# LeadRDRK/ZPack

Measured on AMD Instinct MI355X. Metric: decompressed GiB/s over all entries; % HBM roofline, higher is better.
Workload: dtype u8; 1 GPU; c2_lz4_64k; entries_per_gpu=100000, entries_total=100000, archive_image_bytes_this_rank=3543588472, archive_image_bytes_all_ranks=3543588472, method=lz4, level=0, class_mix=70/20/5/5 text/records/random/runs, parallelism=one batch per rank, no data-path collective, rehearsal_one_card=False, frames_by=liblz4/libzstd of the image, reference writer call sequence

## Files before the change

zpack_amd/csrc/lz4_wave.h:

```cpp
#pragma once
#include "zpk_device.h"
#include "xxh3_device.h"
#include "seq_exec.h"

namespace zpk {

__device__ __noinline__ u32 window_word(const u8* a, const u8* lo, const u8* hi)
{
    if (a >= lo && a + 4 <= hi) return ld32(a);
    u32 v = 0;
    #pragma unroll
    for (int i = 0; i < 4; i++) if (a + i >= lo && a + i < hi) v |= (u32)ld8(a + i) << (8 * i);
    return v;
}

struct ByteWindow {
    u32 w;
    const u8* base;
    const u8* lo;
    const u8* hi;

    __device__ __forceinline__ void load(const u8* p, int lane)
    {
        base = (const u8*)((u64)p & ~(u64)3);
        w = window_word(base + 4 * lane, lo, hi);
    }
    __device__ __forceinline__ u32 byte(const u8* p, int lane)
    {
        u64 d = (u64)(p - base);
        if (d >= 256) { load(p, lane); d = (u64)(p - base); }
        u32 word = (u32)__builtin_amdgcn_readlane((int)w, (int)(d >> 2));
        return (word >> (8 * (d & 3))) & 0xFF;
    }
};

struct DecodeOut { int rc; u64 produced; };

struct Lz4Resume { u64 ip_off, op_off, frame_ip_off, frame_op_off; u32 in_blocks, nframes; };

#ifndef LZ4W_SEG
#define LZ4W_SEG 60u
#endif
static_assert(LZ4W_SEG <= 64u, "the visited-position mask of a segment is one 64-bit word");
#define LZ4W_CHUNK (64u * LZ4W_SEG)
#define LZ4W_SLACK 64u
#ifndef LZ4W_RUNIN
#define LZ4W_RUNIN LZ4W_SEG
#endif

#ifndef LZ4W_FIX_CONT
#define LZ4W_FIX_CONT 1
#endif

#ifndef LZ4W_SPLIT_FIRST
#define LZ4W_SPLIT_FIRST 0
#endif
#ifndef LZ4W_NREC
#define LZ4W_NREC 576u
#endif
struct alignas(16) Lz4WaveShared {
    u8  stage[LZ4W_CHUNK + LZ4W_SLACK + 16];
    u16 rec[LZ4W_NREC];
};

struct Lz4Bytes {
    lds_cp8 S;
    const u8* g;
    u32 cbase, cend;
    __device__ __forceinline__ u32 at(u32 pos) const
    {
        if (pos < cend) return lds_ld8(S + (pos - cbase));
        return (u32)ld8(g + pos);
    }
    __device__ __forceinline__ u32 at16(u32 pos) const
    {
        if (pos + 1 < cend) return lds_ld16(S + (pos - cbase));
        return at(pos) | (at(pos + 1) << 8);
    }
};

struct Lz4Tok { u32 next, lit_pos, lit, ml, off, flags; };

__device__ __forceinline__ Lz4Tok lz4_token_at(const Lz4Bytes& B, u32 p, u32 C, bool want_offset)
{
    Lz4Tok t; t.flags = 0; t.ml = 0; t.off = 1;
    const u32 tok = B.at(p);
    u32 q = p + 1, lit = tok >> 4;
    if (lit == 15) {
        u32 b;
        do {
            if (q >= C) { t.flags = 1; t.next = C; t.lit = 0; t.lit_pos = q; return t; }
            b = B.at(q++); lit += b;
        } while (b == 255 && lit < 0x7F000000u);
        if (b == 255) { t.flags = 1; t.next = C; t.lit = 0; t.lit_pos = q; return t; }
    }
    t.lit_pos = q; t.lit = lit;
    if (lit > C - q) { t.flags = 1; t.next = C; return t; }
    q += lit;
    if (q == C) { t.flags = 2; t.next = C; return t; }
    if (C - q < 2) { t.flags = 5; t.next = C; return t; }
    if (want_offset) t.off = B.at16(q);
    q += 2;
    u32 ml = tok & 15;
    if (ml == 15) {
        u32 b;
        do {
            if (q >= C) { t.flags = 5; t.next = C; return t; }
            b = B.at(q++); ml += b;
        } while (b == 255 && ml < 0x7F000000u);
        if (b == 255) { t.flags = 5; t.next = C; return t; }
    }
    t.ml = ml + 4;
    t.next = q;
    return t;
}

struct Lz4Quick { u32 lit_pos, lit, ml, next, off, slow; };
__device__ __forceinline__ u32 lt31(u32 a, u32 b) { return (a - b) >> 31; }
__device__ __forceinline__ Lz4Quick lz4_quick(lds_cp8 S, u32 cbase, u32 p, u32 lim)
{
    const lds_cp8 at = S + (p - cbase);
    const u32 tok = lds_ld8(at), b1 = lds_ld8(at + 1);
    const u32 lit4 = tok >> 4, mlc = tok & 15;
    const u32 le = (lit4 + 1) >> 4, me = (mlc + 1) >> 4;
    const u32 lit = lit4 + (b1 & (0u - le));
    const u32 q = 1 + le + lit;
    const u32 b2 = lds_ld8(at + q + 2);
    Lz4Quick r;
    r.off = lds_ld16(at + q);
    r.lit_pos = p + 1 + le; r.lit = lit;
    r.ml = mlc + 4 + (b2 & (0u - me));
    r.next = p + q + 2 + me;
    r.slow = (le & ((b1 + 1) >> 8)) | (me & ((b2 + 1) >> 8)) | lt31(lim, p + q + 3);
    return r;
}

struct Lz4Walk { u32 exit, flags; u64 m; };
template <bool FIRST>
__device__ __forceinline__ Lz4Walk lz4_walk(const Lz4Bytes& B, bool on, u32 from, u32 seg_start, u32 seg_end, u32 C,
                                            const Lz4Walk& old, u32& entry_out, SeqStats& stt)
{
    (void)stt;
    const u32 lim = B.cend < C ? B.cend : C;
    const i32 seg_len = (i32)(seg_end - seg_start), lim_rel = (i32)(lim - seg_start);
    const lds_cp8 base = B.S + (seg_start - B.cbase);
    const bool start_in = on && (i32)(from - seg_start) < seg_len;
    i32 rp = start_in ? (i32)(from - seg_start) : seg_len;
    bool live = start_in;
    u32 flags = 0, exit_far = from, far = on && !start_in ? 1u : 0u;
    u64 m = 0;
    for (;;) {
        live = live && rp < seg_len;
        const bool inseg = FIRST ? rp >= 0 : true;
        if (!FIRST) {
            live = live && !((u32)(old.m >> (rp & 63)) & 1u);
        }
        if (__builtin_amdgcn_ballot_w64(live) == 0) break;
        SEQ_STAT(if (FIRST) stt.hops_first++; else stt.hops_fix++);
        m |= (u64)((live && inseg) ? 1u : 0u) << (rp & 63);
        const lds_cp8 at = base + rp;
        const u32 tok = lds_ld8(at), b1 = lds_ld8(at + 1);
        const u32 lit4 = tok >> 4, mlc = tok & 15;
        const bool l15 = lit4 == 15, m15 = mlc == 15;
        const u32 q = lit4 + 1 + (l15 ? b1 + 1 : 0u);
        const u32 b2 = lds_ld8(at + q + 2);
        const i32 n2 = rp + (i32)q + 2;
        i32 nx = n2 + (m15 ? 1 : 0);
        const bool slow = (l15 && b1 == 255) || (m15 && b2 == 255) || n2 >= lim_rel;
        if (live && slow) {
            SEQ_STAT(stt.slow_hops++);
            const Lz4Tok tt = lz4_token_at(B, seg_start + (u32)rp, C, false);
            nx = (i32)(tt.next - seg_start);
            if (tt.flags && !inseg) nx = 0;
            else if (tt.flags || nx >= seg_len) { flags |= tt.flags; far = 1; exit_far = tt.next; nx = seg_len; }
        }
        rp = live ? nx : rp;
    }
    Lz4Walk w; w.m = m; w.flags = flags; w.exit = far ? exit_far : seg_start + (u32)rp;
    if (!FIRST && rp < seg_len) {
        const u64 tail = old.m & ~((1ull << (rp & 63)) - 1);
        w.m |= tail;
        w.flags |= old.flags;
        w.exit = old.exit;
    }
    if (!on) w = old;
    entry_out = !FIRST ? from : m ? seg_start + (u32)__ffsll((long long)m) - 1u : w.exit;
    return w;
}

struct Lz4NoEmit { __device__ __forceinline__ int operator()(const SeqBatch&, int, u32) const { return D_OK; } };

template <int COOP = 2, bool EMIT = false, class Emit = Lz4NoEmit>
__device__ inline int lz4_block_wave(Lz4WaveShared& sh, Watchdog& wd, SeqStats& stt, const u8* ip, u32 C, const u8* rd_hi,
                                     u8* dst_lo, u8*& op_io, u8* oend, int lane, Emit emit = Emit())
{
    u8* op = op_io;
    if (C == 0) return D_MALFORMED;
    u32 cpos = 0;
    bool finished = false;
    while (!finished) {
        if (wd.expired()) return D_MALFORMED;
        const u64 tp0 = SEQ_T(); (void)tp0;
        if (cpos >= C) return D_MALFORMED;
        const u32 nst = C - cpos < LZ4W_CHUNK + LZ4W_SLACK ? C - cpos : LZ4W_CHUNK + LZ4W_SLACK;
        const u32 tok_end = C - cpos < LZ4W_CHUNK ? C : cpos + LZ4W_CHUNK;
        wave_mem_fence();
        if (ip + cpos + ((nst + 15u) & ~15u) <= rd_hi) {
            const u8* const g = ip + cpos + 16u * (u32)lane;
            ZPK_LDS u8* const d0 = (ZPK_LDS u8*)sh.stage;
            #pragma unroll
            for (u32 i = 0; i < LZ4W_CHUNK + LZ4W_SLACK; i += WAVE * 16)
                if (i + 16u * (u32)lane < nst) __builtin_amdgcn_global_load_lds((const ZPK_GLOBAL u32*)(g + i), (ZPK_LDS u32*)(d0 + i), 16, 0, 0);
            asm volatile("s_waitcnt vmcnt(0)" ::: "memory");
        } else {
            for (u32 i = (u32)lane * 16; i < nst; i += WAVE * 16) {
                const u8* g = ip + cpos + i;
                if (i + 16 <= nst && g + 16 <= rd_hi) { u128 v = ld128(g); __builtin_memcpy(sh.stage + i, &v, 16); }
                else for (u32 k = i; k < nst && k < i + 16; k++) sh.stage[k] = ld8(ip + cpos + k);
            }
        }
        __builtin_amdgcn_fence(__ATOMIC_ACQ_REL, "workgroup");
        u64 ts = SEQ_T(); (void)ts; SEQ_STAT(stt.t_stage += ts - tp0; stt.chunks++);
        Lz4Bytes B; B.S = to_lds(sh.stage); B.g = ip; B.cbase = cpos; B.cend = cpos + nst;
        const u32 lim = B.cend < C ? B.cend : C;
        const u32 my_start = cpos + (u32)lane * LZ4W_SEG;
        const u32 my_end = my_start + LZ4W_SEG < tok_end ? my_start + LZ4W_SEG : tok_end;
        const bool active = my_start < tok_end;
        u32 my_entry = my_start;
        Lz4Walk w; w.exit = my_start; w.flags = 0; w.m = 0;
        w = lz4_walk<true>(B, active, lane == 0 ? my_start : (my_start - cpos > LZ4W_RUNIN ? my_start - LZ4W_RUNIN : cpos), my_start, my_end, C, w, my_entry, stt);
        SEQ_STAT({ u64 t2 = SEQ_T(); stt.t_walk1 += t2 - ts; ts = t2; });
#if LZ4W_FIX_CONT
        {
            static_assert(sizeof(sh.rec) >= 16 * (WAVE + 1), "65 records of 16 bytes (lane 63 reads a slot nobody uses)");
            const lds_p8 slot = to_lds_rw((u8*)sh.rec) + 16u * (u32)lane;
            const auto pack = [](const Lz4Walk& a) { u128 v; v.lo = a.m; v.hi = ((u64)a.flags << 32) | a.exit; return v; };
            const auto unpack = [](const u128& v) { Lz4Walk a; a.m = v.lo; a.exit = (u32)v.hi; a.flags = (u32)(v.hi >> 32); return a; };
            if (lane == 0) my_entry = w.exit;
            bool on = false;
            for (int iter = 0; iter < 2 * 66;) {
                const bool step2 = iter & 1;
                const u32 s0 = my_start + (step2 ? LZ4W_SEG : 0u);
                const u32 s1 = s0 + LZ4W_SEG < C ? s0 + LZ4W_SEG : C;
                const u32 next_end = s1 + LZ4W_SEG < C ? s1 + LZ4W_SEG : C;
                u32 from; Lz4Walk old;
                wave_mem_fence();
                if (!step2) {
                    SEQ_STAT(stt.fix_iters++);
                    from = (u32)__shfl_up((int)w.exit, 1, 64);
                    on = active && from != my_entry;
                    if (__ballot(on) == 0) break;
                    old = w;
                    lds_st128(slot, pack(w));
                } else {
                    from = w.exit;
                    old = unpack(lds_ld128(slot + 16));
                    wave_mem_fence();
                    lds_st128(slot, pack(w));
                }
                wave_mem_fence();
                u32 unused;
                const Lz4Walk r = lz4_walk<false>(B, on, from, s0, s1, C, old, unused, stt);
                if (!step2) {
                    my_entry = on ? from : my_entry;
                    on = on && r.exit != w.exit && r.exit < next_end && r.exit - cpos < LZ4W_CHUNK;
                    w = r;
                    iter += __ballot(on) != 0 ? 1 : 2;
                } else {
                    const u32 hn = (u32)__shfl_up((int)from, 1, 64);
                    const bool got = ((__ballot(on) << 1) >> lane) & 1;
                    wave_mem_fence();
                    if (on) lds_st128(slot + 16, pack(r));
                    wave_mem_fence();
                    w = unpack(lds_ld128(slot));
                    my_entry = got ? hn : my_entry;
                    iter++;
                }
            }
        }
#else
        for (int iter = 0; iter < 66; iter++) {
            SEQ_STAT(stt.fix_iters++);
            u32 e = (u32)__shfl_up((int)w.exit, 1, 64);
            if (lane == 0) e = cpos;
            const bool changed = active && e != my_entry;
            if (__ballot(changed) == 0) break;
            u32 unused;
            w = lz4_walk<false>(B, changed, e, my_start, my_end, C, w, unused, stt);
            my_entry = changed ? e : my_entry;
        }
#endif
        SEQ_STAT({ u64 t2 = SEQ_T(); stt.t_fix += t2 - ts; ts = t2; });
        if (!active) { w.exit = (u32)__shfl((int)w.exit, 63, 64); }
        const u64 lastmask = __ballot(active);
        const int last_lane = 63 - __clzll((long long)lastmask);
        const u32 chain_exit = (u32)__builtin_amdgcn_readlane((int)w.exit, last_lane);
        const u32 fl = (u32)__ballot(active && (w.flags & 1)) != 0 || (__ballot(active && (w.flags & 1)) >> 32) != 0 ? 1u : 0u;
        if (__ballot(active && (w.flags & 2)) != 0) finished = true;
        const u32 my_nseq = active ? (u32)__popcll(w.m) : 0u;
        const u32 x = wave_scan_add(my_nseq);
        const u32 nseq = (u32)__builtin_amdgcn_readlane((int)x, 63);
        SEQ_STAT({ u64 t2 = SEQ_T(); stt.t_emit += t2 - ts; stt.t_parse += t2 - tp0; });
        const u8* ipb = ip;
        asm volatile("" : "+s"(ipb));
        Lz4Bytes Bb = B; Bb.g = ipb;
        ZPK_LDS u16* const rec = (ZPK_LDS u16*)sh.rec;
        for (u32 b0 = 0, bstep; b0 < nseq; b0 += bstep) {
            bstep = LZ4W_SPLIT_FIRST && b0 < WAVE ? WAVE / 2 : WAVE;
            const u32 bw = b0 % LZ4W_NREC;
            if (bw == 0) {
                wave_mem_fence();
                u64 m = w.m;
                u32 k = x - my_nseq;
                const u32 rel = my_start - cpos;
                while (m) {
                    const u32 b = (u32)__ffsll((long long)m) - 1u;
                    m &= m - 1;
                    if (k - b0 < LZ4W_NREC) rec[k - b0] = (u16)(rel + b);
                    k++;
                }
                if (active && x == nseq && nseq - b0 < LZ4W_NREC)
                    rec[nseq - b0] = (u16)(w.exit - cpos < LZ4W_CHUNK + LZ4W_SLACK ? w.exit - cpos : LZ4W_CHUNK + LZ4W_SLACK);
                wave_mem_fence();
            }
            const int cnt = (int)(nseq - b0 < bstep ? nseq - b0 : bstep);
            const u64 tq0 = SEQ_T(); (void)tq0;
            SeqBatch q; q.lit = ipb; q.lit_lds = SEQ_NO_LDS; q.ll = 0; q.ml = 0; q.off = 1; q.bad = 0;
            u32 tok_pos = cpos;
            if (lane < cnt) {
                const u32 p = cpos + (u32)rec[bw + (u32)lane];
                tok_pos = p;
                const Lz4Quick t = lz4_quick(B.S, B.cbase, p, lim);
                if (!t.slow) {
                    q.lit = ipb + t.lit_pos; q.ll = t.lit; q.ml = t.ml; q.off = t.off;
                } else {
                    const Lz4Tok tt = lz4_token_at(Bb, p, C, true);
                    q.lit = ipb + tt.lit_pos; q.ll = tt.lit; q.ml = tt.ml; q.off = tt.off;
                    if (tt.flags & 1) q.bad = (tt.flags & 4) ? 2u : 1u;
                }
                if (q.ll > (1u << 23)) q.ll = 1u << 23;
                if (q.ml > (1u << 23)) q.ml = 1u << 23;
                const u32 lp = (u32)(q.lit - ipb);
                if (q.ll <= SEQ_OWN_MAX && lp + q.ll <= B.cend) q.lit_lds = lp - B.cbase;
            }
            SEQ_STAT({ u64 t2 = SEQ_T(); stt.t_parse += t2 - tq0; stt.t_tok += t2 - tq0; });
            u32 dead = 0;
            if constexpr (!EMIT) {
                const u32 nx = bw + (u32)cnt;
                const u32 own = tok_pos - cpos;
#ifdef LZ4W_ROOM_OWN_TOKEN
                (void)nx; const u32 nxt = 0u;
#else
                const u32 nxt = (u32)rec[nx == LZ4W_NREC ? 0u : nx];
#endif
                dead = (u32)__builtin_amdgcn_readfirstlane((int)(nxt > own ? nxt : own));
            }
            int rc;
            if constexpr (EMIT) { (void)dead; rc = emit(q, cnt, (u32)(q.lit - ipb)); }
            else rc = seq_exec_batch<true, COOP, SEQ_ASM_LONG_LIT != 0>(q, cnt, op, oend, dst_lo, -1, lane, stt, B.S, to_lds_rw(sh.stage), dead);
            if (rc != D_OK) { op_io = op; return rc; }
        }
        if (fl) return D_MALFORMED;
        if (!finished && chain_exit <= cpos) return D_MALFORMED;
        cpos = chain_exit;
    }
    if (cpos != C) return D_MALFORMED;
    op_io = op;
    return D_OK;
}

template <int COOP = 2>
__device__ inline DecodeOut lz4f_decode_wave(Lz4WaveShared& sh, Watchdog& wd, SeqStats& stt, const u8* src, u64 src_size, const u8* src_lo, const u8* src_hi,
                                             u8* dst, u64 dst_cap, int lane, Lz4Resume* rs = nullptr)
{
    DecodeOut r; r.rc = D_OK; r.produced = 0;
    const u8* ip = src;
    const u8* const iend = src + src_size;
    u8* op = dst;
    u8* const oend = dst + dst_cap;
    bool resume_in_blocks = false, first = true;
    if (rs && (rs->in_blocks || rs->nframes)) {
        ip = src + rs->frame_ip_off; op = dst + rs->frame_op_off;
        resume_in_blocks = rs->in_blocks != 0;
        first = rs->nframes == 0;
    }
    for (;; first = false) {
        if (wd.expired()) { r.rc = D_MALFORMED; return r; }
        if (!first && (ip == iend || op == oend)) break;
        if (rs) { rs->frame_ip_off = (u64)(ip - src); rs->frame_op_off = (u64)(op - dst); if (!resume_in_blocks) rs->in_blocks = 0; }
        if (iend - ip < 7) { r.rc = D_TRUNCATED; r.produced = (u64)(op - dst); return r; }
        const u32 magic = uld32(ip);
        if ((magic & 0xFFFFFFF0u) == 0x184D2A50u) {
            if (iend - ip < 8) { r.rc = D_TRUNCATED; r.produced = (u64)(op - dst); return r; }
            const u64 sz = uld32(ip + 4);
            if ((u64)(iend - ip) - 8 < sz) { r.rc = D_TRUNCATED; r.produced = (u64)(op - dst); return r; }
            ip += 8 + sz;
            if (rs) rs->nframes++;
            continue;
        }
        if (magic != 0x184D2204u) { r.rc = D_MALFORMED; return r; }
        const u32 flg = uld8(ip + 4), bd = uld8(ip + 5);
        const bool indep = (flg >> 5) & 1, bck = (flg >> 4) & 1, has_cs = (flg >> 3) & 1, cck = (flg >> 2) & 1, has_dict = flg & 1;
        if ((flg >> 6) != 1 || (flg & 2)) { r.rc = D_MALFORMED; return r; }
        const u32 hdr = 7 + (has_cs ? 8 : 0) + (has_dict ? 4 : 0);
        if ((u64)(iend - ip) < hdr) { r.rc = D_TRUNCATED; r.produced = (u64)(op - dst); return r; }
        if (bd & 0x8F) { r.rc = D_MALFORMED; return r; }
        const u32 bcode = (bd >> 4) & 7;
        if (bcode < 4) { r.rc = D_MALFORMED; return r; }
        const u64 bmax = (u64)1 << (8 + 2 * bcode);
        u64 content_size = 0;
        if (has_cs) content_size = uni64(ld64(ip + 6));
        {
            u32 h = 0;
            lane0_guard();
            if (lane == 0) h = (xxh32_serial(ip + 4, hdr - 5, 0) >> 8) & 0xFF;
            if (uni(h) != uld8(ip + hdr - 1)) { r.rc = D_MALFORMED; return r; }
        }
        ip += hdr;

        u8* const frame_out = op;
        if (resume_in_blocks) { ip = src + rs->ip_off; op = dst + rs->op_off; resume_in_blocks = false; }
        for (;;) {
            if (wd.expired()) { r.rc = D_MALFORMED; return r; }
            if (rs) { rs->in_blocks = 1; rs->ip_off = (u64)(ip - src); rs->op_off = (u64)(op - dst); }
            if (iend - ip < 4) { r.rc = D_TRUNCATED; r.produced = (u64)(op - dst); return r; }
            const u32 bh = uld32(ip);
            ip += 4;
            if (bh == 0) break;
            const bool raw = bh >> 31;
            const u64 bsz = bh & 0x7FFFFFFFu;
            if (bsz > bmax) { r.rc = D_MALFORMED; return r; }
            if ((u64)(iend - ip) < bsz + (bck ? 4u : 0u)) {
                if (raw && !rs) {
                    u64 n = (u64)(iend - ip); if (n > bsz) n = bsz;
                    bool full = n > (u64)(oend - op);
                    if (full) n = (u64)(oend - op);
                    for (u64 i = (u64)lane * 16; i < n; i += WAVE * 16) gcopy_upto16(op + i, ip + i, (u32)(n - i < 16 ? n - i : 16));
                    op += n;
                    if (full) { r.rc = D_DST_FULL; r.produced = (u64)(op - dst); return r; }
                }
                r.rc = D_TRUNCATED; r.produced = (u64)(op - dst); return r;
            }
// ... 93 lines not shown
```

zpack_amd/csrc/seq_exec.h:

```cpp
#pragma once
#include "zpk_device.h"

namespace zpk {

__device__ __forceinline__ void gcopy_upto16(u8* d, const u8* s, u32 n)
{
    if (n >= 16) { st128(d, ld128(s)); return; }
    if (n & 8) { st64(d, ld64(s)); d += 8; s += 8; }
    if (n & 4) { st32(d, ld32(s)); d += 4; s += 4; }
    if (n & 2) { st16(d, ld16(s)); d += 2; s += 2; }
    if (n & 1) st8(d, ld8(s));
}

struct Copy32 { u128 lo, hi; };

__device__ __forceinline__ Copy32 gload_upto32(const u8* s, u32 n)
{
    Copy32 c; c.lo.lo = c.lo.hi = c.hi.lo = c.hi.hi = 0;
    if (n >= 16)      { c.lo = ld128(s); c.hi = ld128(s + n - 16); }
    else if (n >= 8)  { c.lo.lo = ld64(s); c.hi.lo = ld64(s + n - 8); }
    else if (n >= 4)  { c.lo.lo = ld32(s); c.hi.lo = ld32(s + n - 4); }
    else if (n >= 2)  { c.lo.lo = ld16(s); c.hi.lo = ld16(s + n - 2); }
    else if (n == 1)  { c.lo.lo = ld8(s); }
    return c;
// ... 80 lines not shown
    if (n > 48) gstore_upto16(d + 48, v3, n - 48);
}

__device__ __forceinline__ void gcopy_upto32(u8* d, const u8* s, u32 n)
{
    const Copy32 c = gload_upto32(s, n);
    gstore_upto32(d, c, n);
}

__device__ __forceinline__ const u8* readlane_ptr(const u8* p, int k)
{
    return (const u8*)(((u64)(u32)__builtin_amdgcn_readlane((int)(u32)((u64)p >> 32), k) << 32) |
                       (u32)__builtin_amdgcn_readlane((int)(u32)(u64)p, k));
}

__device__ __forceinline__ u8* shfl_ptr(const u8* p, int k)
{
    return (u8*)(((u64)(u32)__shfl((int)(u32)((u64)p >> 32), k, 64) << 32) | (u32)__shfl((int)(u32)(u64)p, k, 64));
}

__device__ __forceinline__ void coop_copy_rows(u64 mask, u32 n, u8* d, const u8* s, bool pat, u32 period, u64 pv, int lane)
{
    const int g = lane >> 4;
    const u32 sub16 = 16u * (u32)(lane & 15);
    while (mask) {
        int k[4];
        #pragma unroll
        for (int i = 0; i < 4; i++) { k[i] = mask ? __ffsll((long long)mask) - 1 : -1; if (mask) mask &= mask - 1; }
        const int kk = g == 0 ? k[0] : (g == 1 ? k[1] : (g == 2 ? k[2] : k[3]));
        const int from = kk < 0 ? lane : kk;
        const u32 rn_any = (u32)__shfl((int)n, from, 64);
        const u32 rn = kk < 0 ? 0u : rn_any;
        u8* const rd = shfl_ptr(d, from);
        const u8* const rs = shfl_ptr(s, from);
        const bool rpat = __shfl((int)(pat ? 1 : 0), from, 64) != 0;
        const u32 rper = (u32)__shfl((int)period, from, 64);
        u64 x = ((u64)(u32)__shfl((int)(u32)(pv >> 32), from, 64) << 32) | (u32)__shfl((int)(u32)pv, from, 64);
        if (rper < 8u) { x &= 0xFFFFFFFFull; x |= x << 32; }
        if (rper < 4u) { x &= 0x0000FFFF0000FFFFull; x |= x << 16; }
        if (rper < 2u) { x &= 0x00FF00FF00FF00FFull; x |= x << 8; }
        for (u32 c = sub16; __ballot(c < rn) != 0; c += 256u) {
            if (c < rn) {
                u128 v; v.lo = x; v.hi = x;
                if (!rpat) v = gload_upto16(rs + c, rn - c);
                gstore_upto16(rd + c, v, rn - c);
            }
        }
    }
}

__device__ __forceinline__ void seq_coop_round(u64 cm, u32 ml, u32 off, u8* ms, const u8* srcp, const u8* oend, int lane)
{
    const bool mine = (cm >> lane) & 1;
    const bool self_overlap = ml > off;
    const bool pat = mine && self_overlap && off <= 8u && (off & (off - 1u)) == 0u;
    Copy32 cb; cb.lo.lo = cb.lo.hi = cb.hi.lo = cb.hi.hi = 0;
    if (pat) cb = gload_wide32(srcp, off, srcp + 16 <= oend);
    const u64 gm = __ballot(mine && (pat || !self_overlap));
    if (gm) coop_copy_rows(gm, ml, ms, srcp, pat, off, cb.lo.lo, lane);
    u64 rest = cm & ~gm;
    while (rest) {
        const int k = __ffsll((long long)rest) - 1;
        rest &= rest - 1;
        const u32 n = (u32)__builtin_amdgcn_readlane((int)ml, k);
        const u32 koff = (u32)__builtin_amdgcn_readlane((int)off, k);
        u8* p = (u8*)readlane_ptr(ms, k);
        const u8* m = readlane_ptr(srcp, k);
        if (koff >= 16) {
            for (u32 c = (u32)lane * 16; c < koff; c += WAVE * 16) gcopy_upto16(p + c, m + c, koff - c);
            wave_mem_fence();
            for (u32 base = koff; base < n; base += koff) {
                const u32 slab = n - base < koff ? n - base : koff;
                for (u32 c = (u32)lane * 16; c < slab; c += WAVE * 16) gcopy_upto16(p + base + c, p + base - koff + c, slab - c);
                wave_mem_fence();
            }
        } else {
            for (u32 c = lane; c < n; c += WAVE) st8(p + c, ld8(m + c % koff));
        }
    }
}

#ifdef ZPK_STATS
struct SeqStats { u64 t_parse, t_lit, t_dep, t_rounds; u32 rounds, batches, coops, redirects; u64 t_stage, t_walk1, t_fix, t_emit, t_tok; u32 fix_iters, chunks, asm_batches, hops_first, hops_fix, slow_hops;
    u32 r_room, r_piece, r_both, r_straddle, k_lit, k_match, k_so16, k_so1; u64 t_asm, t_dir; u32 b_asm, b_dir; };
#define SEQ_T() __builtin_amdgcn_s_memtime()
#define SEQ_STAT(x) do { x; } while (0)
#else
struct SeqStats { };
#define SEQ_T() 0ull
#define SEQ_STAT(x) do { } while (0)
#endif

#define SEQ_OWN_MAX 32u
#ifndef SEQ_DEP_ROUNDS
#define SEQ_DEP_ROUNDS 4
#endif

#define SEQ_NO_LDS 0xFFFFFFFFu
#ifndef SEQ_ASM_LONG_LIT
#define SEQ_ASM_LONG_LIT 1
#endif
#define SEQ_ASM_PRE 32u
#define SEQ_ASM_SLACK 16u
struct SeqBatch {
    const u8* lit;
    u32 lit_lds;
    u32 ll, ml;
    u32 off;
    u32 bad;
};

template <typename S>
__device__ __forceinline__ u64 seq_dependencies(bool has_match, u32 r_ms, u32 r_me, u32 off, u32 need_len, u64 pending, int lane,
                                                i64& src_out, SeqStats& stt)
{
    (void)stt;
    S src = (S)r_ms - (S)off;
    u64 need = 0;
    const S send0 = src + (S)need_len;
    const bool reads_batch = has_match && send0 > 0;
    if (pending && __ballot(reads_batch) != 0) {
        int inside = -1;
        int klo = 0, khi = 0;
        #pragma unroll
        for (int step = 32; step >= 1; step >>= 1) {
            const u32 a = (u32)__shfl((int)r_me, klo + step - 1, 64);
            const u32 b = (u32)__shfl((int)r_ms, khi + step - 1, 64);
            if ((S)a <= src) klo += step;
            if ((S)b < send0) khi += step;
        }
        if (reads_batch && klo < khi) {
            if (khi > lane) khi = lane;
            const u64 span = (khi >= 64 ? ~0ull : ((1ull << khi) - 1)) & ~((1ull << klo) - 1);
            need = span & pending;
            if (need && (need & (need - 1)) == 0) inside = __ffsll((long long)need) - 1;
        }
        {
            const int probe = inside < 0 ? lane : inside;
            const u32 kms = (u32)__shfl((int)r_ms, probe, 64);
            const u32 knl = (u32)__shfl((int)need_len, probe, 64);
            if (inside >= 0 && !((S)kms <= src && send0 <= (S)kms + (S)knl)) inside = -1;
        }
        #pragma unroll 1
        for (int round = 0; round < SEQ_DEP_ROUNDS; round++) {
            if (__ballot(inside >= 0) == 0) break;
            SEQ_STAT(stt.redirects += (u32)__popcll(__ballot(inside >= 0)));
            const int probe = inside < 0 ? lane : inside;
            const S my_delta = (S)r_ms - src;
            const u32 dlo = (u32)__shfl((int)(u32)(u64)(i64)my_delta, probe, 64);
            const u32 dhi = sizeof(S) == 8 ? (u32)__shfl((int)(u32)((u64)(i64)my_delta >> 32), probe, 64) : 0u;
            const u32 nlo = (u32)__shfl((int)(u32)need, probe, 64), nhi = (u32)__shfl((int)(u32)(need >> 32), probe, 64);
            const int kin = __shfl(inside, probe, 64);
            if (inside >= 0) { src -= sizeof(S) == 8 ? (S)(i64)(((u64)dhi << 32) | dlo) : (S)(i32)dlo; need = ((u64)nhi << 32) | nlo; inside = kin; }
        }
    }
    src_out = (i64)src;
    return need;
}

template <bool NARROW_ONLY = false, int COOP = 2, bool LONG_LIT = false>
__device__ __forceinline__ int seq_exec_batch(const SeqBatch& q, int cnt, u8*& op, u8* oend, const u8* dst_lo, int lit_rle, int lane,
                                              SeqStats& stt, lds_cp8 lit_stage = nullptr, lds_p8 asm_buf = nullptr, u32 asm_cap = 0)
{
    u64 t0 = SEQ_T(); (void)t0; (void)stt;
    const u64 tb = t0; (void)tb;
    SEQ_STAT(stt.batches++);
    const bool act = lane < cnt;
    const u32 ll = act ? q.ll : 0u, ml = act ? q.ml : 0u;
    const u32 x = wave_scan_add(ll + ml);
    const u64 total = (u32)__builtin_amdgcn_readlane((int)x, 63);
    u8* const o = op + (x - (ll + ml));
    u8* const ms = o + ll;
    const bool has_match = act && ml != 0;
    {
        const u64 cap = (u64)(oend - op);
        const bool off_bad = has_match && (q.off == 0 || (u64)q.off > (u64)(ms - dst_lo));
        u32 v = 0;
        if (act) {
            if (q.bad == 1) v = 1;
            else if ((u64)(x - ml) > cap) v = 2;
            else if (q.bad == 2 || off_bad) v = 1;
            else if ((u64)x > cap) v = 2;
        }
        const u64 vm = __ballot(v != 0);
        if (vm != 0) return (u32)__builtin_amdgcn_readlane((int)v, __ffsll((long long)vm) - 1) == 1u ? D_MALFORMED : D_DST_FULL;
    }
    u64 pending = __ballot(has_match);

    const u32 r_ms = (u32)(ms - op), r_me = r_ms + ml;
    const u32 need_len = ml < q.off ? ml : q.off;
    i64 src;
    u64 need;
    if (NARROW_ONLY) need = seq_dependencies<i32>(has_match, r_ms, r_me, q.off, need_len, pending, lane, src, stt);
    else {
        const bool narrow = total < (1u << 30) && __ballot(has_match && q.off >= (1u << 30)) == 0;
        need = narrow ? seq_dependencies<i32>(has_match, r_ms, r_me, q.off, need_len, pending, lane, src, stt)
                      : seq_dependencies<i64>(has_match, r_ms, r_me, q.off, need_len, pending, lane, src, stt);
    }
    const u8* const srcp = op + src;
    const bool self_overlap = ml > need_len;
    const bool coop = has_match && (ml > SEQ_OWN_MAX || self_overlap);
    const bool early = has_match && !coop && src + (i64)need_len <= 0;
    SEQ_STAT({ u64 t1 = SEQ_T(); stt.t_dep += t1 - t0; t0 = t1; });

#ifdef ZPK_STATS
        if (lit_rle < 0 && NARROW_ONLY) {
            const bool fits = total + (SEQ_ASM_PRE + SEQ_ASM_SLACK) <= (u64)asm_cap;
            const u64 kl = __ballot(ll > SEQ_OWN_MAX), km = __ballot(has_match && !self_overlap && ml > SEQ_OWN_MAX);
            const u64 k16 = __ballot(has_match && self_overlap && q.off >= 16u), k1 = __ballot(has_match && self_overlap && q.off < 16u);
            const bool piece = ((LONG_LIT ? 0ull : kl) | km | k16 | k1) != 0;
            if (!fits) { if (piece) stt.r_both++; else stt.r_room++; }
            else {
                if (piece) stt.r_piece++;
                else if (__ballot(has_match && !early && src < 0) != 0 && (u64)(op - dst_lo) < SEQ_ASM_PRE) stt.r_straddle++;
                stt.k_lit += kl != 0; stt.k_match += km != 0; stt.k_so16 += k16 != 0; stt.k_so1 += k1 != 0;
            }
        }
#endif
    if (lit_rle < 0 && total + (SEQ_ASM_PRE + SEQ_ASM_SLACK) <= (u64)asm_cap) {
        const bool straddle = has_match && !early && src < 0;
        const u64 sm = __ballot(straddle);
        if (__ballot(coop || (!LONG_LIT && ll > SEQ_OWN_MAX)) == 0 && (sm == 0 || (u64)(op - dst_lo) >= SEQ_ASM_PRE)) {
            SEQ_STAT(stt.asm_batches++);
            const lds_p8 ob = asm_buf + SEQ_ASM_PRE;
            if (sm != 0 && lane < 2) lds_st128(asm_buf + 16 * lane, ld128(op - SEQ_ASM_PRE + 16 * lane));
            const u32 ln = LONG_LIT && ll > SEQ_OWN_MAX ? 0u : ll;
            Copy32 ca;
            if (q.lit_lds != SEQ_NO_LDS) {
                ca.lo.lo = ca.lo.hi = ca.hi.lo = ca.hi.hi = 0;
                if (ln) { ca.lo = lds_ld128(lit_stage + q.lit_lds); if (ln > 16) ca.hi = lds_ld128(lit_stage + q.lit_lds + (ln - 16)); }
            } else ca = gload_wide32(q.lit, ln, false);
            if (LONG_LIT && ll > SEQ_OWN_MAX) {
                const lds_p8 p = ob + (r_ms - ll);
                for (u32 c = 0; c < ll; c += 16) {
                    const u32 at = c + 16 <= ll ? c : ll - 16;
                    lds_st128(p + at, ld128(q.lit + at));
                }
            }
            const u32 mn = early ? ml : 0u;
            const Copy32 cb = gload_wide32(srcp, mn, srcp + 16 <= oend);
            lds_store_wide32(ob + (r_ms - ll), ca, ln);
            lds_store_wide32(ob + r_ms, cb, mn);
            wave_mem_fence();
            u64 done = ~pending | __ballot(early);
            pending &= ~done;
            u32 guard = 0;
            while (pending) {
                const bool ready = has_match && ((pending >> lane) & 1) && (need & ~done) == 0;
                const u64 rmask = __ballot(ready);
                if (rmask == 0 || ++guard > 70) return D_MALFORMED;
                SEQ_STAT(stt.rounds++);
                if (ready) {
                    const lds_cp8 sp = (lds_cp8)(ob + (i32)src);
                    Copy32 c; c.hi.lo = c.hi.hi = 0;
                    c.lo = lds_ld128(sp);
                    if (ml > 16) c.hi = lds_ld128(sp + (ml - 16));
                    lds_store_wide32(ob + r_ms, c, ml);
                }
                wave_mem_fence();
                done |= rmask;
                pending &= ~rmask;
            }
            const u32 tot = (u32)total;
            for (u32 c = (u32)lane * 16; c < tot; c += WAVE * 16) {
                const u128 v = lds_ld128((lds_cp8)(ob + c));
                if (c + 16 <= tot) st128(op + c, v);
                else gstore_upto16(op + c, v, tot - c);
            }
            wave_mem_fence();
            SEQ_STAT({ stt.t_asm += SEQ_T() - tb; stt.b_asm += (u32)total; });
            op += total;
            return D_OK;
        }
    }

    if (lit_rle >= 0) {
        if (__ballot(ll > SEQ_OWN_MAX) == 0) { for (u32 c = 0; c < ll; c++) st8(o + c, (u8)lit_rle); }
        else {
            for (int k = 0; k < cnt; k++) {
                const u32 n = (u32)__builtin_amdgcn_readlane((int)ll, k);
                u8* p = (u8*)readlane_ptr(o, k);
                for (u32 c = lane; c < n; c += WAVE) st8(p + c, (u8)lit_rle);
            }
        }
        if (early) { const Copy32 cb = gload_wide32(srcp, ml, srcp + 16 <= oend); gstore_wide32(ms, cb, ml); }
    } else {
        const bool long_lit = ll > SEQ_OWN_MAX;
        const u32 ln = long_lit ? 0u : ll, mn = early ? ml : 0u;
        Copy32 ca;
        const bool from_lds = q.lit_lds != SEQ_NO_LDS;
        if (from_lds) {
            ca.lo.lo = ca.lo.hi = ca.hi.lo = ca.hi.hi = 0;
            if (ln) { ca.lo = lds_ld128(lit_stage + q.lit_lds); if (ln > 16) ca.hi = lds_ld128(lit_stage + q.lit_lds + (ln - 16)); }
        } else ca = gload_wide32(q.lit, ln, false);
        const Copy32 cb = gload_wide32(srcp, mn, srcp + 16 <= oend);
        gstore_wide32(o, ca, ln);
        gstore_wide32(ms, cb, mn);
        if constexpr (COOP >= 2) {
            const u64 lm = __ballot(long_lit);
            if (lm) coop_copy_rows(lm, ll, o, q.lit, false, 16u, 0ull, lane);
        } else {
        u64 lm = __ballot(long_lit);
        while (lm) {
            const int k = __ffsll((long long)lm) - 1;
            lm &= lm - 1;
            const u32 n = (u32)__builtin_amdgcn_readlane((int)ll, k);
            u8* p = (u8*)readlane_ptr(o, k);
            const u8* s = readlane_ptr(q.lit, k);
            for (u32 c = (u32)lane * 16; c < n; c += WAVE * 16) gcopy_upto16(p + c, s + c, n - c);
        }
        }
    }
    wave_mem_fence();
    u64 done = ~pending | __ballot(early);
    pending &= ~done;
    SEQ_STAT({ u64 t1 = SEQ_T(); stt.t_lit += t1 - t0; t0 = t1; });

    u32 guard = 0;
    while (pending) {
        const bool ready = has_match && ((pending >> lane) & 1) && (need & ~done) == 0;
        const u64 rmask = __ballot(ready);
        if (rmask == 0 || ++guard > 70) return D_MALFORMED;
        SEQ_STAT(stt.rounds++);
        if (ready && !coop) {
            const Copy32 cb = gload_wide32(srcp, ml, srcp + 16 <= oend);
            gstore_wide32(ms, cb, ml);
        }
        if constexpr (COOP >= 1) {
            const u64 cm = __ballot(ready && coop);
            SEQ_STAT(stt.coops += (u32)__popcll(cm));
            if (cm) seq_coop_round(cm, ml, q.off, ms, srcp, oend, lane);
        } else {
        u64 cm = __ballot(ready && coop);
        SEQ_STAT(stt.coops += (u32)__popcll(cm));
        while (cm) {
            const int k = __ffsll((long long)cm) - 1;
            cm &= cm - 1;
            const u32 n = (u32)__builtin_amdgcn_readlane((int)ml, k);
            const u32 koff = (u32)__builtin_amdgcn_readlane((int)q.off, k);
            u8* p = (u8*)readlane_ptr(ms, k);
            const u8* m = readlane_ptr(srcp, k);
            if (koff >= n) { for (u32 c = (u32)lane * 16; c < n; c += WAVE * 16) gcopy_upto16(p + c, m + c, n - c); }
            else if (koff >= 16) {
                for (u32 c = (u32)lane * 16; c < koff; c += WAVE * 16) gcopy_upto16(p + c, m + c, koff - c);
                wave_mem_fence();
                for (u32 base = koff; base < n; base += koff) {
                    const u32 slab = n - base < koff ? n - base : koff;
                    for (u32 c = (u32)lane * 16; c < slab; c += WAVE * 16) gcopy_upto16(p + base + c, p + base - koff + c, slab - c);
                    wave_mem_fence();
                }
            } else {
                for (u32 c = lane; c < n; c += WAVE) st8(p + c, ld8(m + c % koff));
            }
// ... 13 lines not shown
```

zpack_amd/csrc/zpk_codec.hip:

```cpp
#include <hip/hip_runtime.h>
#include <stdio.h>
#include <stdlib.h>
#include <string.h>
#include <new>
#include <time.h>
#include <pthread.h>
#include <thread>
#include <atomic>
#include <vector>
#include <algorithm>


#include "zpk_device.h"
#include "xxh3_device.h"
#include "xxh3_span.h"
#include "lz4_wave.h"
#include "lx_ring.h"
#ifndef LX_WAVES_PER_SIMD
#define LX_WAVES_PER_SIMD 6
#endif
#include "zstd_wg.h"
#include "zstd_fse4.h"
#include "zstd_ring.h"
#include "lz4_pj.h"
// ... 159 lines not shown

template <bool LDS_KEYS = false>
__device__ __forceinline__ void finish_entry(const zpk_decode_desc& d, zpk_decode_result* res, u32 e, int status, u32 detail,
                                             u64 produced, const u8* out, int lane, lds_p8 sec = nullptr)
{
    u64 h = 0;
    lane0_guard();
    if (status == R_OK) {
        wave_mem_fence();
        h = xxh3_64_wave<LDS_KEYS>(out, d.uncomp_size, lane, sec);
        if (h != d.expect_hash && !(d.flags & ZPK_DF_SKIP_HASH)) status = R_FILE_HASH_MISMATCH;
    }
    lane0_guard();
    if (lane == 0) {
        zpk_decode_result r; r.status = status; r.detail = detail; r.produced = produced; r.hash = h;
        res[e] = r;
    }
}

__global__ __launch_bounds__(256) void k_stored(const u8* __restrict__ src, const zpk_decode_desc* __restrict__ desc,
                                                u8* __restrict__ dst, zpk_decode_result* __restrict__ res,
                                                const u32* __restrict__ list, const u32* __restrict__ counters)
{
    const int lane = lane_id();
    u32 idx;
    if (my_slot(counters, C_NONE, idx)) {
        const u32 e = uni(list[idx]);
        const zpk_decode_desc d = desc[e];
        const u8* in = uni_ptr(src + d.src_offset);
        u8* out = uni_ptr(dst + d.dst_offset);
        const u64 len = uni64(d.uncomp_size);
        u64 h;
        if (len <= 240) {
            for (u64 i = lane; i < len; i += WAVE) st8(out + i, ld8(in + i));
            h = 0;
            lane0_guard();
            if (lane == 0) h = xxh3_short(in, (u32)len);
            h = uni64(h);
        } else {
            Xxh3Wave st; st.init(lane);
            const u64 nblocks = (len - 1) >> 10;
            const u8* q = in + 16 * lane;
            u8* o = out + 16 * lane;
            u128 cur = {0, 0};
            if (nblocks) cur = ld128(q);
            for (u64 b = 0; b < nblocks; b++) {
                u128 nxt = {0, 0};
                if (b + 1 < nblocks) nxt = ld128(q + ((b + 1) << 10));
                st128(o + (b << 10), cur);
                st.block(cur);
                cur = nxt;
            }
            const u64 done = nblocks << 10;
            for (u64 i = done + lane; i < len; i += WAVE) st8(out + i, ld8(in + i));
            const u32 nstripes = (u32)(((len - 1) - done) >> 6);
            h = st.finish(in + done, nstripes, in + len, len, lane);
        }
        int status = R_OK;
        if (!(d.flags & ZPK_DF_SKIP_HASH) && h != d.expect_hash) status = R_FILE_HASH_MISMATCH;
        lane0_guard();
        if (lane == 0) {
            zpk_decode_result r; r.status = status; r.detail = 0; r.produced = len; r.hash = h;
            res[e] = r;
        }
    }
}

__device__ __forceinline__ void lz4_stats_out(u64* __restrict__ dbg, u32 e, const SeqStats& stt, u64 t_all, int lane)
{
#ifdef ZPK_STATS
    if (dbg && lane == 0) {
        u64* g = dbg + (u64)e * 8;
        g[0] = stt.t_parse; g[1] = stt.t_lit; g[2] = stt.t_dep; g[3] = stt.t_rounds;
        g[4] = ((u64)stt.batches << 32) | stt.rounds; g[5] = ((u64)stt.coops << 32) | stt.asm_batches; g[6] = SEQ_T() - t_all;
        g[7] = ((u64)stt.fix_iters << 32) | stt.chunks;
#ifdef ZPK_STATS_PARSE
        g[0] = stt.t_stage; g[1] = stt.t_walk1; g[2] = stt.t_fix; g[3] = stt.t_emit; g[4] = stt.t_tok;
        g[5] = ((u64)stt.hops_first << 32) | stt.hops_fix; g[6] = stt.slow_hops;
#endif
#ifdef ZPK_STATS_ASM
        g[0] = ((u64)stt.batches << 32) | stt.asm_batches; g[1] = ((u64)stt.r_room << 32) | stt.r_piece; g[2] = ((u64)stt.r_both << 32) | stt.r_straddle;
        g[3] = ((u64)stt.k_lit << 32) | stt.k_match; g[4] = ((u64)stt.k_so16 << 32) | stt.k_so1; g[5] = stt.t_asm; g[6] = stt.t_dir;
        g[7] = ((u64)stt.b_asm << 32) | stt.b_dir;
#endif
    }
#else
    (void)dbg; (void)e; (void)stt; (void)t_all; (void)lane;
#endif
}

template <int COOP>
__device__ __forceinline__ void lz4_entry_wave(Lz4WaveShared& shw, const u8* __restrict__ src, const u8* read_lo, const u8* read_hi,
                                               const zpk_decode_desc* __restrict__ desc, u8* dst, zpk_decode_result* __restrict__ res,
                                               u32 e, u32* __restrict__ counters, u64* __restrict__ dbg, u32* __restrict__ retry_list,
                                               u32 wd_scale, int lane)
{
    const zpk_decode_desc d = desc[e];
    const u8* in = uni_ptr(src + d.src_offset);
    u8* out = uni_ptr(dst + d.dst_offset);
    Watchdog wd; wd.arm(uni64(d.comp_size) + uni64(d.dst_capacity), wd_scale);
    SeqStats stt = {};
    const u64 t_all = SEQ_T(); (void)t_all;
    DecodeOut o = lz4f_decode_wave<COOP>(shw, wd, stt, in, uni64(d.comp_size), read_lo, read_hi, out, uni64(d.dst_capacity), lane);
    lz4_stats_out(dbg, e, stt, t_all, lane);
    if (wd.fired && retry_list) {
        lane0_guard();
        if (lane == 0) retry_list[atomicAdd(&counters[C_RETRY_LZ4], 1u)] = e;
        return;
    }
    int status = R_OK;
    if (o.rc == D_MALFORMED) status = R_DECOMPRESS_FAILED;
    else if (o.rc == D_TRUNCATED) status = o.produced < d.dst_capacity ? R_FILE_INCOMPLETE : R_BUFFER_TOO_SMALL;
    else if (o.rc == D_DST_FULL) status = R_BUFFER_TOO_SMALL;
    finish_entry<true>(d, res, e, status, wd.fired ? 0xDEADu : (u32)(-o.rc), o.produced, out, lane, to_lds_rw(shw.stage));
}

__device__ __forceinline__ void lz4_entry_plain(Lz4WaveShared& shw, const u8* __restrict__ src, const u8* read_hi,
                                                const zpk_decode_desc* __restrict__ desc, u8* dst, zpk_decode_result* __restrict__ res,
                                                u32 e, u32* __restrict__ counters, u64* __restrict__ dbg, u32* __restrict__ retry_list,
                                                u32* __restrict__ handed_list, u32 wd_scale, int lane)
{
    const zpk_decode_desc& d = desc[e];
    const u8* in = uni_ptr(src + d.src_offset);
    u8* out = uni_ptr(dst + d.dst_offset);
    Watchdog wd; wd.arm(uni64(d.comp_size) + uni64(d.dst_capacity), wd_scale);
    SeqStats stt = {};
    const u64 t_all = SEQ_T(); (void)t_all;
    const bool done = lz4f_plain_wave<0>(shw, wd, stt, in, uni64(d.comp_size), read_hi, out, uni64(d.dst_capacity), uni64(d.uncomp_size), lane);
    lz4_stats_out(dbg, e, stt, t_all, lane);
    if (!done) {
        lane0_guard();
        if (lane == 0) {
            if (wd.fired) retry_list[atomicAdd(&counters[C_RETRY_LZ4], 1u)] = e;
            else handed_list[atomicAdd(&counters[C_LZ4_HANDED], 1u)] = e;
        }
        return;
    }
    finish_entry<true>(d, res, e, R_OK, 0u, uni64(d.uncomp_size), out, lane, to_lds_rw(shw.stage));
}

__global__ __launch_bounds__(64, 8) void k_lz4_wave(const u8* __restrict__ src, const u8* read_hi,
                                                  const zpk_decode_desc* __restrict__ desc, u8* dst,
                                                  zpk_decode_result* __restrict__ res, const u32* __restrict__ list,
                                                  u32* __restrict__ counters, u32* __restrict__ retry_list, u32* __restrict__ handed_list
#ifdef ZPK_DEVELOPER
                                                  , u64* __restrict__ dbg, u32 wd_scale
#endif
                                                  )
{
#ifndef ZPK_DEVELOPER
    const u32 wd_scale = 1u;
    u64* const dbg = nullptr;
#endif
    const int lane = lane_id();
    __shared__ Lz4WaveShared shw;
    u32 idx;
    if (my_slot(counters, C_LZ4, idx))
        lz4_entry_plain(shw, src, read_hi, desc, dst, res, uni(list[idx]), counters, dbg, retry_list, handed_list, wd_scale, lane);
}

#ifdef ZPK_DEVELOPER
__global__ __launch_bounds__(256) void k_lz4_hand_all(const u32* __restrict__ list, u32* __restrict__ counters, u32* __restrict__ handed_list)
{
    const u64 i = (u64)blockIdx.x * blockDim.x + threadIdx.x;
    if (i < counters[C_LZ4]) handed_list[atomicAdd(&counters[C_LZ4_HANDED], 1u)] = list[i];
}
// ... 1787 lines not shown
```

Before: 697.8 GiB/s.

## Assemble oversized LZ4 batches in a reusable tail region of the staging buffer

Batches whose output does not fit the dead room ahead of the next token in the LDS stage can now be assembled in a fixed tail region of the stage (offset 2384, up to 1536 bytes). That region is used only when the chunk was DMA-staged. It lets more batches take the LDS assembly path with coalesced 16-byte stores instead of the slower direct global path. The cost is that the overwritten compressed bytes are re-fetched from global into LDS before the next batch, which adds extra loads and a vmcnt wait. It also adds risk if a later token still reads the clobbered region before the restore.

```diff
diff --git a/zpack_amd/csrc/lz4_wave.h b/zpack_amd/csrc/lz4_wave.h
--- a/zpack_amd/csrc/lz4_wave.h
+++ b/zpack_amd/csrc/lz4_wave.h
@@ -58,9 +58,14 @@
 #ifndef LZ4W_NREC
 #define LZ4W_NREC 576u
 #endif
+#define LZ4W_TAIL_AT 2384u
+#define LZ4W_TAIL_CAP 1536u
+static_assert(LZ4W_TAIL_AT % 16u == 0 && LZ4W_TAIL_AT + LZ4W_TAIL_CAP <= LZ4W_CHUNK + LZ4W_SLACK + 16u && LZ4W_TAIL_CAP <= LZ4W_TAIL_AT,
+              "the tail room lies inside the stage, on a 16-byte piece of the staging DMA, behind every batch that takes it");
 struct alignas(16) Lz4WaveShared {
     u8  stage[LZ4W_CHUNK + LZ4W_SLACK + 16];
     u16 rec[LZ4W_NREC];
+    u16 tail_cap[8];
 };
 
 struct Lz4Bytes {
@@ -205,7 +210,9 @@
         const u32 nst = C - cpos < LZ4W_CHUNK + LZ4W_SLACK ? C - cpos : LZ4W_CHUNK + LZ4W_SLACK;
         const u32 tok_end = C - cpos < LZ4W_CHUNK ? C : cpos + LZ4W_CHUNK;
         wave_mem_fence();
-        if (ip + cpos + ((nst + 15u) & ~15u) <= rd_hi) {
+        const bool dma_staged = ip + cpos + ((nst + 15u) & ~15u) <= rd_hi;
+        *(ZPK_LDS u32*)sh.tail_cap = dma_staged ? LZ4W_TAIL_CAP : 0u;
+        if (dma_staged) {
             const u8* const g = ip + cpos + 16u * (u32)lane;
             ZPK_LDS u8* const d0 = (ZPK_LDS u8*)sh.stage;
             #pragma unroll
@@ -305,6 +312,7 @@
         asm volatile("" : "+s"(ipb));
         Lz4Bytes Bb = B; Bb.g = ipb;
         ZPK_LDS u16* const rec = (ZPK_LDS u16*)sh.rec;
+        u32 tail_pending = 0;
         for (u32 b0 = 0, bstep; b0 < nseq; b0 += bstep) {
             bstep = LZ4W_SPLIT_FIRST && b0 < WAVE ? WAVE / 2 : WAVE;
             const u32 bw = b0 % LZ4W_NREC;
@@ -322,6 +330,22 @@
                 if (active && x == nseq && nseq - b0 < LZ4W_NREC)
                     rec[nseq - b0] = (u16)(w.exit - cpos < LZ4W_CHUNK + LZ4W_SLACK ? w.exit - cpos : LZ4W_CHUNK + LZ4W_SLACK);
                 wave_mem_fence();
+            }
+            if (!EMIT && tail_pending != 0) {
+                const u64 tr0 = SEQ_T(); (void)tr0;
+                asm volatile("s_waitcnt lgkmcnt(0)" ::: "memory");
+                const u32 upto = LZ4W_TAIL_AT + tail_pending;
+                const u32 end = nst < upto ? nst : upto;
+                const u32 at = LZ4W_TAIL_AT + 16u * (u32)lane;
+                const u8* const g = ipb + cpos + at;
+                ZPK_LDS u8* const d0 = (ZPK_LDS u8*)sh.stage + LZ4W_TAIL_AT;
+                static_assert(LZ4W_TAIL_CAP <= 2u * WAVE * 16u, "two pieces of 1 KiB cover the tail room");
+                if (at < end) __builtin_amdgcn_global_load_lds((const ZPK_GLOBAL u32*)g, (ZPK_LDS u32*)d0, 16, 0, 0);
+                if (at + WAVE * 16u < end) __builtin_amdgcn_global_load_lds((const ZPK_GLOBAL u32*)g, (ZPK_LDS u32*)d0, 16, WAVE * 16, 0);
+                asm volatile("s_waitcnt vmcnt(0)" ::: "memory");
+                __builtin_amdgcn_fence(__ATOMIC_ACQ_REL, "workgroup");
+                tail_pending = 0;
+                SEQ_STAT(stt.t_tail += SEQ_T() - tr0);
             }
             const int cnt = (int)(nseq - b0 < bstep ? nseq - b0 : bstep);
             const u64 tq0 = SEQ_T(); (void)tq0;
@@ -344,7 +368,7 @@
                 if (q.ll <= SEQ_OWN_MAX && lp + q.ll <= B.cend) q.lit_lds = lp - B.cbase;
             }
             SEQ_STAT({ u64 t2 = SEQ_T(); stt.t_parse += t2 - tq0; stt.t_tok += t2 - tq0; });
-            u32 dead = 0;
+            u32 dead = 0, tail_cap = 0;
             if constexpr (!EMIT) {
                 const u32 nx = bw + (u32)cnt;
                 const u32 own = tok_pos - cpos;
@@ -353,11 +377,17 @@
 #else
                 const u32 nxt = (u32)rec[nx == LZ4W_NREC ? 0u : nx];
 #endif
-                dead = (u32)__builtin_amdgcn_readfirstlane((int)(nxt > own ? nxt : own));
+                const u32 tcap = (u32)((ZPK_LDS u16*)sh.tail_cap)[nx == LZ4W_NREC ? 1u : 0u];
+                const u32 pk = (u32)__builtin_amdgcn_readfirstlane((int)((nxt > own ? nxt : own) | (tcap << 16)));
+                dead = pk & 0xFFFFu; tail_cap = pk >> 16;
             }
             int rc;
             if constexpr (EMIT) { (void)dead; rc = emit(q, cnt, (u32)(q.lit - ipb)); }
-            else rc = seq_exec_batch<true, COOP, SEQ_ASM_LONG_LIT != 0>(q, cnt, op, oend, dst_lo, -1, lane, stt, B.S, to_lds_rw(sh.stage), dead);
+            else {
+                const auto restore = [&](u32 need) { tail_pending = need; };
+                rc = seq_exec_batch<true, COOP, SEQ_ASM_LONG_LIT != 0>(q, cnt, op, oend, dst_lo, -1, lane, stt, B.S, to_lds_rw(sh.stage), dead,
+                                                                       to_lds_rw(sh.stage) + LZ4W_TAIL_AT, tail_cap, restore);
+            }
             if (rc != D_OK) { op_io = op; return rc; }
         }
         if (fl) return D_MALFORMED;
diff --git a/zpack_amd/csrc/seq_exec.h b/zpack_amd/csrc/seq_exec.h
--- a/zpack_amd/csrc/seq_exec.h
+++ b/zpack_amd/csrc/seq_exec.h
@@ -186,7 +186,7 @@
 
 #ifdef ZPK_STATS
 struct SeqStats { u64 t_parse, t_lit, t_dep, t_rounds; u32 rounds, batches, coops, redirects; u64 t_stage, t_walk1, t_fix, t_emit, t_tok; u32 fix_iters, chunks, asm_batches, hops_first, hops_fix, slow_hops;
-    u32 r_room, r_piece, r_both, r_straddle, k_lit, k_match, k_so16, k_so1; u64 t_asm, t_dir; u32 b_asm, b_dir; };
+    u32 r_room, r_piece, r_both, r_straddle, k_lit, k_match, k_so16, k_so1; u64 t_asm, t_dir; u32 b_asm, b_dir; u64 t_tail; u32 b_tail, n_tail; };
 #define SEQ_T() __builtin_amdgcn_s_memtime()
 #define SEQ_STAT(x) do { x; } while (0)
 #else
@@ -262,9 +262,11 @@
     return need;
 }
 
-template <bool NARROW_ONLY = false, int COOP = 2, bool LONG_LIT = false>
+struct SeqNoAlt { __device__ __forceinline__ void operator()(u32) const { } };
+template <bool NARROW_ONLY = false, int COOP = 2, bool LONG_LIT = false, class AltDone = SeqNoAlt>
 __device__ __forceinline__ int seq_exec_batch(const SeqBatch& q, int cnt, u8*& op, u8* oend, const u8* dst_lo, int lit_rle, int lane,
-                                              SeqStats& stt, lds_cp8 lit_stage = nullptr, lds_p8 asm_buf = nullptr, u32 asm_cap = 0)
+                                              SeqStats& stt, lds_cp8 lit_stage = nullptr, lds_p8 asm_buf = nullptr, u32 asm_cap = 0,
+                                              lds_p8 alt_buf = nullptr, u32 alt_cap = 0, AltDone alt_done = AltDone())
 {
     u64 t0 = SEQ_T(); (void)t0; (void)stt;
     const u64 tb = t0; (void)tb;
@@ -321,13 +323,17 @@
             }
         }
 #endif
-    if (lit_rle < 0 && total + (SEQ_ASM_PRE + SEQ_ASM_SLACK) <= (u64)asm_cap) {
+    const bool use_alt = total + (SEQ_ASM_PRE + SEQ_ASM_SLACK) > (u64)asm_cap;
+    if (lit_rle < 0 && total + (SEQ_ASM_PRE + SEQ_ASM_SLACK) <= (u64)(use_alt ? alt_cap : asm_cap)) {
         const bool straddle = has_match && !early && src < 0;
         const u64 sm = __ballot(straddle);
         if (__ballot(coop || (!LONG_LIT && ll > SEQ_OWN_MAX)) == 0 && (sm == 0 || (u64)(op - dst_lo) >= SEQ_ASM_PRE)) {
             SEQ_STAT(stt.asm_batches++);
-            const lds_p8 ob = asm_buf + SEQ_ASM_PRE;
-            if (sm != 0 && lane < 2) lds_st128(asm_buf + 16 * lane, ld128(op - SEQ_ASM_PRE + 16 * lane));
+            const lds_p8 ab0 = use_alt ? alt_buf : asm_buf;
+            #define SEQ_AB() ([&]() { lds_p8 a_ = ab0; if (alt_cap != 0) asm("" : "+s"(a_)); return a_; }())
+            #define ob (SEQ_AB() + SEQ_ASM_PRE)
+            #define ab SEQ_AB()
+            if (sm != 0 && lane < 2) lds_st128(ab + 16 * lane, ld128(op - SEQ_ASM_PRE + 16 * lane));
             const u32 ln = LONG_LIT && ll > SEQ_OWN_MAX ? 0u : ll;
             Copy32 ca;
             if (q.lit_lds != SEQ_NO_LDS) {
@@ -372,7 +378,11 @@
                 else gstore_upto16(op + c, v, tot - c);
             }
             wave_mem_fence();
-            SEQ_STAT({ stt.t_asm += SEQ_T() - tb; stt.b_asm += (u32)total; });
+            SEQ_STAT({ if (ab0 != asm_buf) { stt.t_tail += SEQ_T() - tb; stt.b_tail += (u32)total; stt.n_tail++; } else { stt.t_asm += SEQ_T() - tb; stt.b_asm += (u32)total; } });
+            if (alt_cap != 0 && ab != asm_buf) alt_done((u32)total + (SEQ_ASM_PRE + SEQ_ASM_SLACK));
+            #undef ob
+            #undef ab
+            #undef SEQ_AB
             op += total;
             return D_OK;
         }
diff --git a/zpack_amd/csrc/zpk_codec.hip b/zpack_amd/csrc/zpk_codec.hip
--- a/zpack_amd/csrc/zpk_codec.hip
+++ b/zpack_amd/csrc/zpk_codec.hip
@@ -265,6 +265,9 @@
         g[0] = ((u64)stt.batches << 32) | stt.asm_batches; g[1] = ((u64)stt.r_room << 32) | stt.r_piece; g[2] = ((u64)stt.r_both << 32) | stt.r_straddle;
         g[3] = ((u64)stt.k_lit << 32) | stt.k_match; g[4] = ((u64)stt.k_so16 << 32) | stt.k_so1; g[5] = stt.t_asm; g[6] = stt.t_dir;
         g[7] = ((u64)stt.b_asm << 32) | stt.b_dir;
+        g[3] = ((u64)(stt.k_lit & 0xFFFFu) << 48) | ((u64)(stt.k_match & 0xFFFFu) << 32) | ((stt.k_so16 & 0xFFFFu) << 16) | (stt.k_so1 & 0xFFFFu);
+        g[4] = ((u64)stt.n_tail << 32) | stt.b_tail;
+        g[2] = ((u64)(stt.r_both & 0xFFFFu) << 48) | ((u64)(stt.r_straddle & 0xFFFFu) << 32) | (u32)(stt.t_tail > 0xFFFFFFFFull ? 0xFFFFFFFFull : stt.t_tail);
 #endif
     }
 #else
```

Result: no change. 693.3 GiB/s (-0.6%).
